# pierluigiferrari/ssd_keras

Measured on NVIDIA H100. Metric: SSD300 images/sec (fwd+decode), higher is better.
Workload: dtype bf16x3 (bf16 hi+lo operands, 3 wgmma MMAs per product, fp32 accumulate)

## Files before the change

include/ssdk.h:

```cpp
#ifndef SSDK_H_
#define SSDK_H_

#include <stddef.h>
#include <stdint.h>

#ifdef __cplusplus
extern "C" {
#endif

#define SSDK_VERSION 100

typedef enum {
  SSDK_OK = 0,
  SSDK_ERR_INVALID = -1,
  SSDK_ERR_CUDA = -2,
  SSDK_ERR_UNSUPPORTED = -3,
  SSDK_ERR_NOMEM = -4,
  SSDK_ERR_DEGENERATE = -5
} ssdk_status;

typedef enum { SSDK_COORDS_CENTROIDS = 0, SSDK_COORDS_CORNERS = 1, SSDK_COORDS_MINMAX = 2 } ssdk_coords;

typedef struct ssdk_ctx ssdk_ctx;
typedef struct ssdk_encoder ssdk_encoder;
// ... 150 lines not shown

typedef struct {
  int batch;
  int img_height, img_width, img_channels;
  int n_classes_total;
  int n_layers;
  const ssdk_layer_desc* layers;
  int precision;
  const float* anchors_f32;
  float variances[4];
  int training;
} ssdk_model_desc;

int ssdk_l2_normalize(ssdk_ctx* ctx, const float* x_dev, long long rows, int C, const float* gamma_dev, float* out_dev, void* stream);

int ssdk_conv2d_fwd(ssdk_ctx* ctx, const float* x_dev, int B, int H, int W, int Cin, const float* kernel_hwio_host,
                    const float* bias_host , int Cout, int kh, int kw, int stride, int dilation,
                    int pad_t, int pad_l, int pad_b, int pad_r, int act , int precision, float* y_dev, void* stream);
int ssdk_maxpool(ssdk_ctx* ctx, const float* x_dev, int B, int H, int W, int C, int kh, int kw, int stride,
                 int pad_t, int pad_l, int pad_b, int pad_r, float* y_dev, void* stream);

int ssdk_schedule_preview(int n_layers, const int* kind, const int* grid, const int* input, int R, int sm_count,
                          unsigned char* out_on_side, int* out_from, int* out_grid_cap);

int ssdk_model_create(ssdk_ctx* ctx, const ssdk_model_desc* desc, ssdk_model** out);
int ssdk_model_destroy(ssdk_model* m);
int ssdk_model_num_priors(const ssdk_model* m, int* out_P);
int ssdk_model_layer_shape(const ssdk_model* m, int layer, int* out_h, int* out_w, int* out_c);
int ssdk_model_forward(ssdk_model* m, const float* images_dev, float* y_pred_dev, void* stream);
int ssdk_model_read_layer(ssdk_model* m, int layer, float* out_dev, void* stream);
int ssdk_model_flops(const ssdk_model* m, double* out_algorithmic, double* out_issued);
int ssdk_model_set_timing(ssdk_model* m, int enable);
int ssdk_model_last_conv_ms(ssdk_model* m, float* out_ms);

enum ssdk_plan_kernel {
  SSDK_PLAN_NONE = 0,
  SSDK_PLAN_GEMM = 1,
  SSDK_PLAN_IM2COL_GEMM = 2,
  SSDK_PLAN_FIRST_TC = 3,
  SSDK_PLAN_DIRECT = 4
};
enum ssdk_plan_epilogue { SSDK_PLAN_EPI_SPLIT = 0, SSDK_PLAN_EPI_F32 = 1, SSDK_PLAN_EPI_ATOMIC = 2, SSDK_PLAN_EPI_HEAD = 3 };
typedef struct ssdk_layer_plan {
  int kernel;
  int bn;
  int split;
  int stages;
  int kblocks;
  int n_tiles_m, n_tiles_n;
  int grid;
  int k_split;
  int epilogue;
  int head_fused;
  int im2col_vec8;
} ssdk_layer_plan;
int ssdk_model_layer_plan(const ssdk_model* m, int layer, ssdk_layer_plan* out);

typedef struct ssdk_trainer ssdk_trainer;
int ssdk_trainer_create(ssdk_model* m, float* flat_grad_dev , ssdk_trainer** out);
int ssdk_trainer_destroy(ssdk_trainer* t);
int ssdk_trainer_num_params(const ssdk_trainer* t, long long* out_n);
int ssdk_trainer_param_span(const ssdk_trainer* t, int layer, int which, long long* out_offset, long long* out_count);
float* ssdk_trainer_grad_buffer(ssdk_trainer* t);
int ssdk_train_backward(ssdk_trainer* t, const float* y_true_dev, const float* y_pred_dev, int neg_pos_ratio, int n_neg_min,
                        float alpha, float* out_loss_dev , void* stream);
int ssdk_train_backward_begin(ssdk_trainer* t, const float* y_true_dev, const float* y_pred_dev, int neg_pos_ratio, int n_neg_min,
// ... 37 lines not shown
```

ssd_keras_b200/_ffi.py:

```python
import ctypes as C
import os
import threading

import numpy as np

_HERE = os.path.dirname(os.path.abspath(__file__))
_LIB_PATH = os.path.join(_HERE, '_lib', 'libssdk.so')

SSDK_OK = 0
SSDK_ERR_INVALID = -1
SSDK_ERR_CUDA = -2
SSDK_ERR_UNSUPPORTED = -3
SSDK_ERR_NOMEM = -4
SSDK_ERR_DEGENERATE = -5

COORDS = {'centroids': 0, 'corners': 1, 'minmax': 2}
BORDER_D = {'half': 0, 'include': 1, 'exclude': -1}

c_int_p = C.POINTER(C.c_int)
c_float_p = C.POINTER(C.c_float)
c_double_p = C.POINTER(C.c_double)


class AnchorCfg(C.Structure):
# ... 122 lines not shown
        L.ssdk_iou.argtypes = [vp, vp, C.c_int, vp, C.c_int, C.c_int, C.c_int, C.c_int, vp, vp]
        L.ssdk_decode.argtypes = [vp, C.POINTER(DecodeCfg), vp, C.c_int, vp, vp, vp, vp]
        L.ssdk_nms.argtypes = [vp, vp, vp, C.c_int, C.c_int, C.c_double, C.c_double, C.c_int, C.c_int, vp, vp, vp, vp]
        L.ssdk_ssd_loss_fwd.argtypes = [vp, vp, vp, C.c_int, C.c_int, C.c_int, C.c_int, C.c_int, C.c_float, vp, vp, vp]
        L.ssdk_ssd_loss_bwd.argtypes = [vp, vp, vp, C.c_int, C.c_int, C.c_int, C.c_int, C.c_int, C.c_float, vp, vp, vp]
        L.ssdk_ssd_loss_fwd_bwd.argtypes = [vp, vp, vp, C.c_int, C.c_int, C.c_int, C.c_int, C.c_int, C.c_float, vp, vp, vp, vp, vp]
        L.ssdk_ssd_loss_ws_layout.argtypes = [C.c_int, C.c_int, C.POINTER(LossWsLayout)]
        L.ssdk_ssd_loss_phase.argtypes = [vp, C.c_int, vp, vp, C.c_int, C.c_int, C.c_int, C.c_int, C.c_int, C.c_float, vp, C.c_int, vp,
                                          C.c_int, vp, vp, vp, vp, vp]
        for name in ('ssdk_ssd_loss_fwd_bwd', 'ssdk_ssd_loss_ws_layout', 'ssdk_ssd_loss_phase'):
            getattr(L, name).restype = C.c_int
        L.ssdk_eval_match.argtypes = [vp, C.c_int, vp, C.c_int, vp, vp, vp, vp, vp, vp, vp, vp, C.c_double, C.c_int, vp, vp, vp]
        L.ssdk_eval_cumsum.argtypes = [vp, vp, vp, vp, C.c_int, vp, vp, vp]
        L.ssdk_eval_match.restype = C.c_int
        L.ssdk_eval_cumsum.restype = C.c_int
        L.ssdk_assemble_batch.argtypes = [vp, vp, C.c_int, vp, C.c_int, C.c_int, vp, C.c_int, vp, vp, vp, vp]
        L.ssdk_assemble_batch.restype = C.c_int
        L.ssdk_l2_normalize.argtypes = [vp, vp, C.c_longlong, C.c_int, vp, vp, vp]
        L.ssdk_l2_normalize.restype = C.c_int
        L.ssdk_conv2d_fwd.argtypes = [vp, vp] + [C.c_int] * 4 + [vp, vp] + [C.c_int] * 11 + [vp, vp]
        L.ssdk_conv2d_fwd.restype = C.c_int
        L.ssdk_maxpool.argtypes = [vp, vp] + [C.c_int] * 11 + [vp, vp]
        L.ssdk_maxpool.restype = C.c_int
        if hasattr(L, 'ssdk_model_create'):
            L.ssdk_model_create.argtypes = [vp, C.POINTER(ModelDesc), C.POINTER(vp)]
            L.ssdk_model_destroy.argtypes = [vp]
            L.ssdk_model_num_priors.argtypes = [vp, c_int_p]
            L.ssdk_model_layer_shape.argtypes = [vp, C.c_int, c_int_p, c_int_p, c_int_p]
            L.ssdk_model_forward.argtypes = [vp, vp, vp, vp]
            L.ssdk_model_read_layer.argtypes = [vp, C.c_int, vp, vp]
            L.ssdk_model_flops.argtypes = [vp, c_double_p, c_double_p]
            L.ssdk_model_set_timing.argtypes = [vp, C.c_int]
            L.ssdk_model_last_conv_ms.argtypes = [vp, c_float_p]
            L.ssdk_model_layer_plan.argtypes = [vp, C.c_int, C.POINTER(LayerPlan)]
            L.ssdk_model_layer_plan.restype = C.c_int
        if hasattr(L, 'ssdk_trainer_create'):
            L.ssdk_trainer_create.argtypes = [vp, vp, C.POINTER(vp)]
            L.ssdk_trainer_destroy.argtypes = [vp]
            L.ssdk_trainer_num_params.argtypes = [vp, C.POINTER(C.c_longlong)]
            L.ssdk_trainer_param_span.argtypes = [vp, C.c_int, C.c_int, C.POINTER(C.c_longlong), C.POINTER(C.c_longlong)]
            L.ssdk_trainer_grad_buffer.argtypes = [vp]
            L.ssdk_trainer_grad_buffer.restype = vp
            L.ssdk_train_backward.argtypes = [vp, vp, vp, C.c_int, C.c_int, C.c_float, vp, vp]
            L.ssdk_train_apply_adam.argtypes = [vp, C.c_float, C.c_float, C.c_float, C.c_float, C.c_float, C.c_float, C.c_int, vp]
            L.ssdk_train_apply_adam.restype = C.c_int
            L.ssdk_trainer_read_bn_stats.argtypes = [vp, C.c_int, vp, vp, vp]
            L.ssdk_trainer_read_bn_stats.restype = C.c_int
            L.ssdk_train_backward_dy.argtypes = [vp, vp, vp]
            L.ssdk_train_backward_dy.restype = C.c_int
            L.ssdk_train_backward_begin.argtypes = [vp, vp, vp, C.c_int, C.c_int, C.c_float, vp, vp]
            L.ssdk_train_backward_begin.restype = C.c_int
            L.ssdk_train_backward_layers.argtypes = [vp, vp, C.c_int, C.c_int, vp]
            L.ssdk_train_backward_layers.restype = C.c_int
            L.ssdk_train_apply.argtypes = [vp, C.c_float, C.c_float, C.c_float, C.c_float, vp]
            L.ssdk_trainer_read_params.argtypes = [vp, vp, vp]
            L.ssdk_trainer_layer_plan.argtypes = [vp, C.c_int, C.POINTER(TrainerLayerPlan)]
            L.ssdk_trainer_layer_plan.restype = C.c_int
            for name in ('ssdk_trainer_create', 'ssdk_trainer_destroy', 'ssdk_trainer_num_params', 'ssdk_trainer_param_span',
                         'ssdk_train_backward', 'ssdk_train_apply', 'ssdk_trainer_read_params'):
                getattr(L, name).restype = C.c_int
        for name in ('ssdk_ctx_create', 'ssdk_ctx_destroy', 'ssdk_anchors_count', 'ssdk_anchors_generate',
                     'ssdk_encoder_create', 'ssdk_encoder_destroy', 'ssdk_encode', 'ssdk_encode_f64', 'ssdk_encode_dev', 'ssdk_iou_matrix', 'ssdk_iou', 'ssdk_decode',
                     'ssdk_nms', 'ssdk_ssd_loss_fwd', 'ssdk_ssd_loss_bwd'):
            getattr(L, name).restype = C.c_int
        _lib = L
    return _lib
# ... 87 lines not shown
```

ssd_keras_b200/csrc/conv.cu:

```cuda
#include "conv.cuh"
#include "tc.cuh"
#include <cudaTypedefs.h>
#include <cmath>
#include <cstdlib>
#include <cstring>
#include <algorithm>
#include <vector>

namespace ssdk {

static PFN_cuTensorMapEncodeTiled_v12000 g_encode = nullptr;

int tma_init() {
  if (g_encode) return SSDK_OK;
  void* fn = nullptr;
  cudaDriverEntryPointQueryResult qres;
  SSDK_CHECK_CUDA(cudaGetDriverEntryPoint("cuTensorMapEncodeTiled", &fn, cudaEnableDefault, &qres));
  if (qres != cudaDriverEntryPointSuccess || !fn) { set_error("cuTensorMapEncodeTiled is not available in this driver"); return SSDK_ERR_CUDA; }
  g_encode = reinterpret_cast<PFN_cuTensorMapEncodeTiled_v12000>(fn);
  return SSDK_OK;
}

int make_tmap_2d(CUtensorMap* out, const void* base, uint64_t inner, uint64_t rows, uint64_t row_stride_bytes,
                 uint32_t box_inner, uint32_t box_rows) {
// ... 84 lines not shown
    constexpr int kMaxCol = 256;
    const int c_lo = bx * CP4;
    const int k_lo = c_lo >> 5, k_hi = (c_lo + CP4 - 1) >> 5;
    if (c_lo + CP4 > kMaxCol) break;
    float v0[32], v1[32];
    ld_acc32(arow + k_lo * 32, v0);
    if (k_hi != k_lo) ld_acc32(arow + k_hi * 32, v1);
    float e[CP4];
#pragma unroll
    for (int r = 0; r < CP4; ++r) {
      const int col = c_lo + r;
      e[r] = (((col >> 5) == k_lo) ? v0[col & 31] : v1[col & 31]) + s_bias[col];
    }
    float mx = e[0];
#pragma unroll
    for (int r = 1; r < C; ++r) mx = fmaxf(mx, e[r]);
    float sum = 0.f;
#pragma unroll
    for (int r = 0; r < C; ++r) { e[r] = expf(e[r] - mx); sum += e[r]; }
    const float inv = 1.0f / sum;
    const int prior = args.head_prior_off + pix * args.head_nb + bx;
    float* dst = args.out_f32 + ((size_t)n * args.head_P + prior) * RW;
    const float4 an = __ldg(reinterpret_cast<const float4*>(args.head_anchors) + prior);
#pragma unroll
    for (int r = 0; r < C; ++r) dst[r] = e[r] * inv;
#pragma unroll
    for (int r = C; r < CP4; ++r) dst[r] = e[r];
    dst[C + 4] = an.x; dst[C + 5] = an.y; dst[C + 6] = an.z; dst[C + 7] = an.w;
    dst[C + 8] = args.head_var[0]; dst[C + 9] = args.head_var[1]; dst[C + 10] = args.head_var[2]; dst[C + 11] = args.head_var[3];
  }
}

template <bool BWD>
__device__ __forceinline__ void epi_split(const ConvArgs& args, const float* acc, int ncols, size_t o, const float* sb,
                                          const float* ss, const float* sh) {
  if (!BWD && !args.bn_scale && args.act == SSDK_ACT_RELU && args.out_lo) {
    for (int c0 = 0; c0 < ncols; c0 += 32) {
      float vr[32];
      ld_acc32(acc + c0, vr);
#pragma unroll
      for (int g2 = 0; g2 < 2; ++g2) {
        uint32_t ph[8], pl[8];
#pragma unroll
        for (int h = 0; h < 2; ++h) {
          const int g = g2 * 2 + h;
          if (c0 + g * 8 < ncols) {
            const float4 b0 = *reinterpret_cast<const float4*>(sb + c0 + g * 8);
            const float4 b1 = *reinterpret_cast<const float4*>(sb + c0 + g * 8 + 4);
            const float bb[8] = {b0.x, b0.y, b0.z, b0.w, b1.x, b1.y, b1.z, b1.w};
#pragma unroll
            for (int j = 0; j < 4; ++j) {
              const float f0 = fmaxf(vr[g * 8 + j * 2] + bb[j * 2], 0.f);
              const float f1 = fmaxf(vr[g * 8 + j * 2 + 1] + bb[j * 2 + 1], 0.f);
              const __nv_bfloat162 hh = __floats2bfloat162_rn(f0, f1);
              const uint32_t hp = *reinterpret_cast<const uint32_t*>(&hh);
              const __nv_bfloat162 ll = __floats2bfloat162_rn(f0 - __uint_as_float(hp << 16), f1 - __uint_as_float(hp & 0xffff0000u));
              ph[h * 4 + j] = hp; pl[h * 4 + j] = *reinterpret_cast<const uint32_t*>(&ll);
            }
          }
        }
        const int cA = c0 + g2 * 16;
        {
          if (cA < ncols) {
            *reinterpret_cast<uint4*>(args.out_hi + o + cA) = make_uint4(ph[0], ph[1], ph[2], ph[3]);
            *reinterpret_cast<uint4*>(args.out_lo + o + cA) = make_uint4(pl[0], pl[1], pl[2], pl[3]);
          }
          if (cA + 8 < ncols) {
            *reinterpret_cast<uint4*>(args.out_hi + o + cA + 8) = make_uint4(ph[4], ph[5], ph[6], ph[7]);
            *reinterpret_cast<uint4*>(args.out_lo + o + cA + 8) = make_uint4(pl[4], pl[5], pl[6], pl[7]);
          }
        }
      }
    }
    return;
  }
  for (int c0 = 0; c0 < ncols; c0 += 32) {
    float vr[32];
    ld_acc32(acc + c0, vr);
#pragma unroll
    for (int g = 0; g < 4; ++g) {
      if (c0 + g * 8 < ncols) {
        uint32_t ph[4], pl[4];
        uint4 mk = make_uint4(0x3f803f80u, 0x3f803f80u, 0x3f803f80u, 0x3f803f80u), oh = make_uint4(0, 0, 0, 0), ol = oh;
        if (BWD) {
          if (args.mask_hi) mk = *reinterpret_cast<const uint4*>(args.mask_hi + o + c0 + g * 8);
          if (args.accumulate) {
            oh = *reinterpret_cast<const uint4*>(args.out_hi + o + c0 + g * 8);
            if (args.out_lo) ol = *reinterpret_cast<const uint4*>(args.out_lo + o + c0 + g * 8);
          }
        }
        const uint32_t mkw[4] = {mk.x, mk.y, mk.z, mk.w}, ohw[4] = {oh.x, oh.y, oh.z, oh.w}, olw[4] = {ol.x, ol.y, ol.z, ol.w};
#pragma unroll
        for (int j = 0; j < 4; ++j) {
          float f[2];
#pragma unroll
          for (int e = 0; e < 2; ++e) {
            const int col = c0 + g * 8 + j * 2 + e;
            float xv = vr[g * 8 + j * 2 + e] + sb[col];
            if (args.bn_scale) xv = xv * ss[col] + sh[col];
            xv = apply_act(xv, args.act);
            if (BWD) {
              if (!(__uint_as_float(((mkw[j] >> (e * 16)) & 0xffffu) << 16) > 0.f)) xv = 0.f;
              xv += __uint_as_float(((ohw[j] >> (e * 16)) & 0xffffu) << 16) + __uint_as_float(((olw[j] >> (e * 16)) & 0xffffu) << 16);
            }
            f[e] = xv;
          }
          __nv_bfloat16 h0 = __float2bfloat16_rn(f[0]), h1 = __float2bfloat16_rn(f[1]);
          __nv_bfloat16 l0 = __float2bfloat16_rn(f[0] - __bfloat162float(h0));
          __nv_bfloat16 l1 = __float2bfloat16_rn(f[1] - __bfloat162float(h1));
          ph[j] = (uint32_t)__bfloat16_as_ushort(h0) | ((uint32_t)__bfloat16_as_ushort(h1) << 16);
          pl[j] = (uint32_t)__bfloat16_as_ushort(l0) | ((uint32_t)__bfloat16_as_ushort(l1) << 16);
        }
        *reinterpret_cast<uint4*>(args.out_hi + o + c0 + g * 8) = make_uint4(ph[0], ph[1], ph[2], ph[3]);
        if (args.out_lo) *reinterpret_cast<uint4*>(args.out_lo + o + c0 + g * 8) = make_uint4(pl[0], pl[1], pl[2], pl[3]);
      }
    }
  }
}

enum { kSingle = 0, kSplitXS = 2 };
template <int BN, int MODE>
__global__ void __launch_bounds__(256, 1)
conv_wgmma_kernel(const __grid_constant__ CUtensorMap tm_a_hi, const __grid_constant__ CUtensorMap tm_a_lo,
                  const __grid_constant__ CUtensorMap tm_b_hi, const __grid_constant__ CUtensorMap tm_b_lo,
                  const __grid_constant__ ConvArgs args) {
  extern __shared__ unsigned char smem_dyn[];
  const uint32_t smem_base = (smem_u32(smem_dyn) + 1023u) & ~1023u;
  unsigned char* smem_al = smem_dyn + (smem_base - smem_u32(smem_dyn));
  const int tid = threadIdx.x, wg = tid >> 7, warp = tid >> 5, lane = tid & 31;
  constexpr bool split = MODE == kSplitXS;
  const int S = args.stages;
  constexpr uint32_t kBTile = (uint32_t)BN * kBK * 2;
  const uint32_t b_off = (uint32_t)kATile * (split ? 2u : 1u);
  const uint32_t stage = b_off + kBTile * (split ? 2u : 1u);
  const uint32_t ring = max(stage * (uint32_t)S, ((uint32_t)kBM * (BN + kAccPad) + 32u) * 4u);
  const uint32_t bar_base = smem_base + ring;
  auto full = [&](uint32_t s) { return bar_base + 8u * s; };
  auto empty = [&](uint32_t s) { return bar_base + 8u * ((uint32_t)S + s); };
  float* s_acc = reinterpret_cast<float*>(smem_al);
  float* s_bias = reinterpret_cast<float*>(smem_al + ring + 256);
  float* s_scale = s_bias + BN;
  float* s_shift = s_scale + BN;

  if (tid == 0) {
    prefetch_tmap(&tm_a_hi); prefetch_tmap(&tm_b_hi);
    if (split) { prefetch_tmap(&tm_a_lo); prefetch_tmap(&tm_b_lo); }
    for (int s = 0; s < S; ++s) { mbar_init(full(s), 1); mbar_init(empty(s), 8); }
    asm volatile("fence.mbarrier_init.release.cluster;" ::: "memory");
  }
  __syncthreads();

  const int KS = args.k_split > 1 ? args.k_split : 1;
  const int total_tiles = args.n_tiles_m * args.n_tiles_n * KS;
  uint32_t g = 0;
  float acc[BN / 2], accx[split ? BN / 2 : 1];
  for (int t = blockIdx.x; t < total_tiles; t += gridDim.x) {
    const int tt = t / KS, ks = t - tt * KS;
    const int m0 = args.tile_list[tt / args.n_tiles_n] * kBM;
    const int n0 = (tt % args.n_tiles_n) * BN;
    const int kb0 = KS > 1 ? ks * args.kb_per : 0;
    const int kb1 = KS > 1 ? min(args.kblocks, kb0 + args.kb_per) : args.kblocks;
    const int nkb = kb1 - kb0, nk = args.KH * args.KW * nkb;
    for (int i = tid; i < BN; i += blockDim.x) {
      const int col = n0 + i;
      s_bias[i] = (args.bias && col < args.cout) ? args.bias[col] : 0.f;
      if (args.bn_scale) { s_scale[i] = col < args.cout ? args.bn_scale[col] : 0.f; s_shift[i] = col < args.cout ? args.bn_shift[col] : 0.f; }
    }
    auto issue = [&](int i) {
      const uint32_t gi = g + (uint32_t)i, s = gi % (uint32_t)S;
      mbar_wait(empty(s), ((gi / (uint32_t)S) & 1u) ^ 1u);
      const int tap = i / nkb, kb = kb0 + (i - tap * nkb), kh = tap / args.KW, kw = tap - kh * args.KW;
      const int row = m0 + args.row_shift[kh] + kw * args.kw_rows;
      const int kcol = (tap * args.kblocks + kb) * kBK + args.b_k_offset;
      const uint32_t dst = smem_base + stage * s;
      mbar_expect_tx(full(s), stage);
      tma_load_2d(dst, &tm_a_hi, kb * kBK, row, full(s));
      tma_load_2d(dst + b_off, &tm_b_hi, kcol, n0, full(s));
      if (split) {
        tma_load_2d(dst + kATile, &tm_a_lo, kb * kBK, row, full(s));
        tma_load_2d(dst + b_off + kBTile, &tm_b_lo, kcol, n0, full(s));
      }
    };
    auto release = [&](int j) {
      __syncwarp();
      if (lane == 0) mbar_arrive(empty((g + (uint32_t)j) % (uint32_t)S));
      if (tid == 0 && j + S < nk) issue(j + S);
    };
    if (tid == 0)
      for (int i = 0; i < min(S, nk); ++i) issue(i);
    wgmma_fence_acc(acc);
    wgmma_fence_acc(accx);
    for (int i = 0; i < nk; ++i) {
      const uint32_t gi = g + (uint32_t)i, s = gi % (uint32_t)S;
      mbar_wait(full(s), (gi / (uint32_t)S) & 1u);
      const uint32_t a_hi = smem_base + stage * s + (uint32_t)wg * (kATile / 2), b_hi = smem_base + stage * s + b_off;
      constexpr uint64_t kDesc = wgmma_desc_hi(16);
      wgmma_fence();
#pragma unroll
      for (int k = 0; k < 4; ++k) {
        const uint32_t sc = (i | k) ? 1u : 0u;
        const uint64_t da = wgmma_desc(kDesc, a_hi + 32u * k), db = wgmma_desc(kDesc, b_hi + 32u * k);
        Wgmma<BN, 0, 0>::mma(acc, da, db, sc);
        if constexpr (split) {
          Wgmma<BN, 0, 0>::mma(accx, da, wgmma_desc(kDesc, b_hi + kBTile + 32u * k), sc);
          Wgmma<BN, 0, 0>::mma(accx, wgmma_desc(kDesc, a_hi + kATile + 32u * k), db, 1u);
        }
      }
      wgmma_commit();
      wgmma_wait<1>();
      if (i > 0) release(i - 1);
    }
    wgmma_wait<0>();
    wgmma_fence_acc(acc);
    wgmma_fence_acc(accx);
    if (nk > 0) release(nk - 1);
    g += (uint32_t)nk;
    if constexpr (split) {
#pragma unroll
      for (int j = 0; j < BN / 2; ++j) acc[j] += accx[j];
    }

    __syncthreads();
    store_acc_tile<BN>(acc, s_acc, wg, warp, lane);
    __syncthreads();
    const int r = tid & (kBM - 1), half = tid >> 7;
    const int v = m0 + r;
    bool valid = v < args.M_total;
    int n = 0, y = 0, x = 0;
    if (valid) {
      n = v / args.rows_per_img;
      const int rr = v - n * args.rows_per_img;
      y = rr / args.in_Wp;
      x = rr - y * args.in_Wp;
      valid = (y < args.Ho) && (x < args.Wo);
    }
    const float* arow = s_acc + (size_t)r * (BN + kAccPad);
    const int ncols = min(BN, args.cout - n0);
    const int h0 = half * (BN / 2), nh = min(BN / 2, ncols - h0);
    if (valid && args.epi == EPI_HEAD) {
      if (half == 0) {
        const int C = args.head_C, CP4 = C + 4, RW = C + 12;
        const int pix = y * args.Wo + x;
        if (CP4 == 25 && args.head_nb <= 8) {
          epi_head_fixed<25>(args, arow, n, pix, s_bias);
        } else {
          for (int bx = 0; bx < args.head_nb; ++bx) {
            const int c_lo = bx * CP4;
            float mx = -INFINITY;
            for (int c = c_lo; c < c_lo + C; ++c) mx = fmaxf(mx, arow[c] + s_bias[c]);
            float sum = 0.f;
            for (int c = c_lo; c < c_lo + C; ++c) sum += expf(arow[c] + s_bias[c] - mx);
            const int prior = args.head_prior_off + pix * args.head_nb + bx;
            float* dst = args.out_f32 + ((size_t)n * args.head_P + prior) * RW;
            for (int rc = 0; rc < CP4; ++rc) {
              const float val = arow[c_lo + rc] + s_bias[c_lo + rc];
              dst[rc] = rc < C ? expf(val - mx) / sum : val;
            }
            const float4 an = __ldg(reinterpret_cast<const float4*>(args.head_anchors) + prior);
            dst[C + 4] = an.x; dst[C + 5] = an.y; dst[C + 6] = an.z; dst[C + 7] = an.w;
            dst[C + 8] = args.head_var[0]; dst[C + 9] = args.head_var[1]; dst[C + 10] = args.head_var[2]; dst[C + 11] = args.head_var[3];
          }
        }
      }
    } else if (valid && nh > 0) {
      if (args.epi == EPI_SPLIT) {
        const size_t o = (((size_t)n * args.out_Hp + (y + args.out_pad)) * args.out_Wp + (x + args.out_pad)) * args.out_Cs + n0 + h0;
        if (args.mask_hi || args.accumulate) epi_split<true>(args, arow + h0, nh, o, s_bias + h0, s_scale + h0, s_shift + h0);
        else epi_split<false>(args, arow + h0, nh, o, s_bias + h0, s_scale + h0, s_shift + h0);
      } else if (args.epi == EPI_ATOMIC) {
        float* dstp = args.out_f32 + (size_t)v * args.out_ld + args.out_col_off + n0 + h0;
        for (int j = 0; j < nh; ++j) atomicAdd(dstp + j, arow[h0 + j]);
      } else {
        const size_t o = (((size_t)n * args.Ho + y) * args.Wo + x) * (size_t)args.cout + n0 + h0;
        for (int j = 0; j < nh; ++j) args.out_f32[o + j] = apply_act(arow[h0 + j] + s_bias[h0 + j], args.act);
      }
    }
    fence_proxy_async();
    __syncthreads();
  }
}

template <int BN, int MODE>
static int launch_conv_bn(const ConvLaunch& L, int grid, cudaStream_t stream) {
  static bool attr_set = false;
  if (!attr_set) {
    SSDK_CHECK_CUDA(cudaFuncSetAttribute(conv_wgmma_kernel<BN, MODE>, cudaFuncAttributeMaxDynamicSharedMemorySize, 227 * 1024));
    attr_set = true;
  }
  conv_wgmma_kernel<BN, MODE><<<grid, 256, L.smem, stream>>>(L.a_hi, L.a_lo, L.b_hi, L.b_lo, L.args);
  return SSDK_OK;
}

int launch_conv(ssdk_ctx* ctx, const ConvLaunch& L, cudaStream_t stream, int grid_cap) {
  const int grid = grid_cap > 0 ? std::max(1, std::min(L.grid, grid_cap)) : L.grid;
  const bool split = L.args.split != 0;
  SSDK_REQUIRE(!split || L.args.acc_split, "internal: bf16x3 conv plans carry the cross-term accumulator");
  SSDK_REQUIRE(split || L.args.BN != 160, "internal: 160-wide conv tiles are for bf16x3 predictor heads");
  int rc;
  switch (L.args.BN) {
    case 64: rc = split ? launch_conv_bn<64, kSplitXS>(L, grid, stream) : launch_conv_bn<64, kSingle>(L, grid, stream); break;
    case 128: rc = split ? launch_conv_bn<128, kSplitXS>(L, grid, stream) : launch_conv_bn<128, kSingle>(L, grid, stream); break;
    case 160: rc = launch_conv_bn<160, kSplitXS>(L, grid, stream); break;
    case 256:
      SSDK_REQUIRE(!split, "internal: 256-wide conv tiles have no cross-term accumulator");
      rc = launch_conv_bn<256, kSingle>(L, grid, stream);
      break;
    default: set_error("internal: conv tile width %d", L.args.BN); return SSDK_ERR_INVALID;
  }
  if (rc) return rc;
  SSDK_COUNT_LAUNCH(ctx);
  SSDK_CHECK_CUDA(cudaGetLastError());
  return SSDK_OK;
}

__device__ __forceinline__ void split_store(const ActBuf& o, size_t idx, float v) {
  __nv_bfloat16 h = __float2bfloat16_rn(v);
  o.hi[idx] = h;
  if (o.lo) o.lo[idx] = __float2bfloat16_rn(v - __bfloat162float(h));
}
__device__ __forceinline__ float split_load(const ActBuf& a, size_t idx) {
  float v = __bfloat162float(a.hi[idx]);
  if (a.lo) v += __bfloat162float(a.lo[idx]);
// ... 304 lines not shown
            const uint32_t off = (uint32_t)(tap >> 4) * kATile + (uint32_t)r * 128u + ((uint32_t)(((tap >> 1) & 7) ^ (r & 7)) << 4) + (uint32_t)(tap & 1) * 8u;
            *reinterpret_cast<uint2*>(a_dst + off) = w[j];
          }
        }
      }
    }
    fence_proxy_async();
    __syncthreads();
    {
      constexpr uint64_t kDesc = wgmma_desc_hi(16);
      wgmma_fence_acc(acc);
      wgmma_fence();
#pragma unroll
      for (int ks = 0; ks < KB * 4; ++ks) {
        const int kb = ks >> 2, k = ks & 3;
        const uint32_t ah = a_base + (uint32_t)kb * kATile + (uint32_t)wg * (kATile / 2) + 32u * k;
        const uint32_t bh = b_base + (uint32_t)kb * b_block + 32u * k;
        const uint64_t da = wgmma_desc(kDesc, ah), db = wgmma_desc(kDesc, bh);
        Wgmma<BN, 0, 0>::mma(acc, da, db, ks ? 1u : 0u);
        if constexpr (split) {
          Wgmma<BN, 0, 0>::mma(acc, da, wgmma_desc(kDesc, bh + b_plane), 1u);
          Wgmma<BN, 0, 0>::mma(acc, wgmma_desc(kDesc, ah + a_plane), db, 1u);
        }
      }
      wgmma_commit();
      wgmma_wait<0>();
      wgmma_fence_acc(acc);
    }
    store_acc_tile<BN>(acc, s_acc, wg, warp, lane);
    __syncthreads();
    const int h0 = plane * (BN / 2), nh = min(BN / 2, fa.epi.cout - h0);
    if (valid && nh > 0) {
      const size_t o = (((size_t)n * fa.epi.out_Hp + (y + fa.epi.out_pad)) * fa.epi.out_Wp + (x + fa.epi.out_pad)) * fa.epi.out_Cs + h0;
      epi_split<false>(fa.epi, s_acc + (size_t)r * (BN + kAccPad) + h0, nh, o, s_bias + h0, s_scale + h0, s_shift + h0);
    }
    __syncthreads();
  }
}

void first_weight_image(const float* hwio, int taps, int cin, int cout, int BN, int kblocks, std::vector<uint16_t>& hi, std::vector<uint16_t>& lo) {
  hi.assign((size_t)kblocks * BN * 64, 0); lo.assign((size_t)kblocks * BN * 64, 0);
  auto f2bf = [](float f) { uint32_t u; memcpy(&u, &f, 4); if ((u & 0x7f800000u) == 0x7f800000u) return (uint16_t)(u >> 16);
                            u += 0x7fffu + ((u >> 16) & 1u); return (uint16_t)(u >> 16); };
  auto bf2f = [](uint16_t h) { uint32_t u = (uint32_t)h << 16; float f; memcpy(&f, &u, 4); return f; };
  for (int o = 0; o < cout; ++o)
    for (int t = 0; t < taps; ++t)
      for (int c = 0; c < cin; ++c) {
        const int k = t * 4 + c, kb = k >> 6, kk = k & 63;
        const size_t byte = (size_t)kb * BN * 128 + (size_t)o * 128 + ((size_t)((kk >> 3) ^ (o & 7)) << 4) + (size_t)(kk & 7) * 2;
        const float w = hwio[((size_t)t * cin + c) * cout + o];
        const uint16_t h = f2bf(w);
        hi[byte / 2] = h; lo[byte / 2] = f2bf(w - bf2f(h));
      }
}

bool first_border_ok(const ActBuf& in, int kh, int kw, int dil, int pad_t, int pad_l) {
  return in.pad >= pad_t && in.pad >= pad_l && in.pad >= (kh - 1) * dil - pad_t && in.pad >= (kw - 1) * dil - pad_l;
}
int first_tc_supported(int taps, int cin, int cout) { return cin <= 4 && taps * 4 <= 128 && cout % 8 == 0 && cout <= 128; }

template <int BN, int KB, bool SPLIT>
static int launch_first_bn(const FirstArgs& fa, int grid, size_t smem, cudaStream_t stream) {
  static bool attr_set = false;
  if (!attr_set) {
    SSDK_CHECK_CUDA(cudaFuncSetAttribute(conv_first_kernel<BN, KB, SPLIT>, cudaFuncAttributeMaxDynamicSharedMemorySize, 227 * 1024));
    attr_set = true;
  }
// ... 307 lines not shown
```

ssd_keras_b200/csrc/model.cu:

```cuda
#include "model.cuh"

using namespace ssdk;

namespace {

void pack_weights(const LayerPlan& L, int cin, int cout, int taps, int kblocks, bool im2col, int Ctot,
                  std::vector<uint16_t>& hi, std::vector<uint16_t>& lo, std::vector<float>& bias) {
  const ssdk_layer_desc& d = L.d;
  const size_t Krow = im2col ? (size_t)kblocks * 64 : (size_t)taps * kblocks * 64;
  hi.assign((size_t)cout * Krow, 0); lo.assign((size_t)cout * Krow, 0);
  bias.assign(cout, 0.f);
  const bool head = d.op == SSDK_OP_HEAD;
  const int nb = d.n_boxes;
  const int c_conf = head ? nb * Ctot : cout;
  const int c_loc = head ? nb * 4 : 0;
  for (int o = 0; o < cout; ++o) {
    const float* ker; int oc, ocn;
    if (!head) { ker = d.kernel; oc = o; ocn = c_conf; bias[o] = d.bias ? d.bias[o] : 0.f; }
    else {
      const int b = o / (Ctot + 4), r = o % (Ctot + 4);
      if (r < Ctot) { ker = d.kernel; oc = b * Ctot + r; ocn = c_conf; bias[o] = d.bias ? d.bias[oc] : 0.f; }
      else { ker = d.kernel2; oc = b * 4 + (r - Ctot); ocn = c_loc; bias[o] = d.bias2 ? d.bias2[oc] : 0.f; }
    }
    for (int t = 0; t < taps; ++t)
// ... 424 lines not shown
  const ConvArgs& a = L.launch.args;
  out->kernel = L.im2col ? SSDK_PLAN_IM2COL_GEMM : SSDK_PLAN_GEMM;
  out->bn = a.BN; out->split = a.split; out->stages = a.stages; out->kblocks = a.kblocks;
  out->n_tiles_m = a.n_tiles_m; out->n_tiles_n = a.n_tiles_n; out->grid = L.launch.grid; out->k_split = a.k_split > 1 ? a.k_split : 1;
  out->epilogue = a.epi; out->head_fused = L.head_fused ? 1 : 0;
  out->im2col_vec8 = L.im2col && L.im2col_vec8 ? 1 : 0;
  return SSDK_OK;
}

extern "C" int ssdk_model_flops(const ssdk_model* m, double* algo, double* issued) {
  SSDK_REQUIRE(m, "ssdk_model_flops: NULL model");
  if (algo) *algo = m->flops_algo;
  if (issued) *issued = m->flops_issued;
  return SSDK_OK;
}

extern "C" int ssdk_model_set_timing(ssdk_model* m, int enable) {
  SSDK_REQUIRE(m, "ssdk_model_set_timing: NULL model");
  m->timing = enable ? 1 : 0;
  return SSDK_OK;
}

extern "C" int ssdk_model_last_conv_ms(ssdk_model* m, float* out_ms) {
  SSDK_REQUIRE(m && out_ms, "ssdk_model_last_conv_ms: NULL argument");
  float total = 0.f;
  for (auto& L : m->layers) {
    if (!L.ev0 || L.direct) continue;
    SSDK_CHECK_CUDA(cudaEventSynchronize(L.ev1));
    float ms = 0.f;
    SSDK_CHECK_CUDA(cudaEventElapsedTime(&ms, L.ev0, L.ev1));
    total += ms;
  }
  *out_ms = total;
  return SSDK_OK;
}

extern "C" int ssdk_model_forward(ssdk_model* m, const float* images_dev, float* y_pred_dev, void* stream_) {
  SSDK_REQUIRE(m && images_dev, "ssdk_model_forward: NULL argument");
  SSDK_REQUIRE(m->P == 0 || y_pred_dev, "ssdk_model_forward: y_pred_dev is NULL");
  cudaStream_t main_stream = (cudaStream_t)stream_;
  ssdk_ctx* ctx = m->ctx;
  int rc;
  const bool overlap = m->overlap_from >= 0 && !m->timing;
  int issued[2] = {0, 0}, seen[2] = {0, 0}, side_used = 0;
  std::vector<int>& pos = m->issue_pos;
  pos.assign(m->layers.size(), 0);
  for (size_t i = 0; i < m->layers.size(); ++i) {
    LayerPlan& L = m->layers[i];
    const ssdk_layer_desc& d = L.d;
    const int sx = overlap && m->on_side[i] ? 1 : 0;
    cudaStream_t stream = sx ? m->side : main_stream;
    int cap = 0;
    if (overlap) {
      if (d.op != SSDK_OP_INPUT && d.input >= 0) {
        const int sy = m->on_side[d.input] ? 1 : 0;
        const bool first_side = sx == 1 && !side_used;
        if ((sy != sx && pos[d.input] > seen[sx]) || first_side) {
          cudaStream_t other = sx ? main_stream : m->side;
          SSDK_CHECK_CUDA(cudaEventRecord(m->dep_ev[i], other));
          SSDK_CHECK_CUDA(cudaStreamWaitEvent(stream, m->dep_ev[i], 0));
          seen[sx] = issued[sx ^ 1];
        }
      }
      if (sx) side_used = 1;
      pos[i] = ++issued[sx];
      if (!sx && side_used) cap = m->grid_cap;
// ... 135 lines not shown
```

ssd_keras_b200/models/_graph.py:

```python
import ctypes as C

import numpy as np

from .. import _ffi
from ..keras_layers.keras_layer_DecodeDetections import DecodeDetections
from ..keras_layers.keras_layer_DecodeDetectionsFast import DecodeDetectionsFast
from ._keras_api import KerasTrainingMixin


class _LayerInfo:
    def __init__(self, name, output_shape):
        self.name = name
        self.output_shape = output_shape


class Spec:

    def __init__(self, name, op, inp=None, cout=0, k=(1, 1), stride=1, dilation=1, pad=(0, 0, 0, 0), act=_ffi.ACT_NONE,
                 n_boxes=0, bn=None, params=None):
        self.name, self.op, self.inp, self.cout = name, op, inp, cout
        self.kh, self.kw = k
        self.stride, self.dilation, self.pad, self.act, self.n_boxes = stride, dilation, pad, act, n_boxes
        self.bn = bn
        self.params = params or {}
# ... 390 lines not shown
                yield item[0] if isinstance(item, (tuple, list)) else item
        outs = [r.numpy().copy() for r in self.predict_stream(images())]
        if not outs:
            raise ValueError('predict_generator: the generator yielded no batch')
        return np.concatenate(outs, axis=0)

    def predict(self, x, batch_size=None):
        x = np.asarray(x, dtype=np.float32)
        bs = batch_size or x.shape[0]
        outs = [r.numpy().copy() for r in self.predict_stream(x[i:i + bs] for i in range(0, x.shape[0], bs))]
        return np.concatenate(outs, axis=0)

    def read_layer(self, name, batch):
        import torch
        i = self.index[name]
        h, w, c = self._shapes[i]
        out = torch.empty((batch, h, w, c), dtype=torch.float32, device='cuda')
        _ffi.check(_ffi.lib().ssdk_model_read_layer(self._plan(batch)['handle'], i, _ffi.dptr(out), _ffi.stream_ptr()))
        return out.cpu().numpy()

    def flops(self, batch):
        a, b = C.c_double(), C.c_double()
        _ffi.check(_ffi.lib().ssdk_model_flops(self._plan(batch)['handle'], C.byref(a), C.byref(b)))
        return a.value, b.value

    def set_timing(self, batch, enable=True):
        _ffi.check(_ffi.lib().ssdk_model_set_timing(self._plan(batch)['handle'], 1 if enable else 0))

    def last_conv_ms(self, batch):
        v = C.c_float()
        _ffi.check(_ffi.lib().ssdk_model_last_conv_ms(self._plan(batch)['handle'], C.byref(v)))
        return v.value


def resolve_box_args(n_predictor_layers, min_scale, max_scale, scales, aspect_ratios_global, aspect_ratios_per_layer,
                     two_boxes_for_ar1, steps, offsets, variances):
    if aspect_ratios_global is None and aspect_ratios_per_layer is None:
        raise ValueError("`aspect_ratios_global` and `aspect_ratios_per_layer` cannot both be None. At least one needs to be specified.")
    if aspect_ratios_per_layer:
        if len(aspect_ratios_per_layer) != n_predictor_layers:
            raise ValueError("It must be either aspect_ratios_per_layer is None or len(aspect_ratios_per_layer) == {}, but "
                             "len(aspect_ratios_per_layer) == {}.".format(n_predictor_layers, len(aspect_ratios_per_layer)))
    if (min_scale is None or max_scale is None) and scales is None:
        raise ValueError("Either `min_scale` and `max_scale` or `scales` need to be specified.")
    if scales:
        if len(scales) != n_predictor_layers + 1:
            raise ValueError("It must be either scales is None or len(scales) == {}, but len(scales) == {}."
                             .format(n_predictor_layers + 1, len(scales)))
    else:
        scales = np.linspace(min_scale, max_scale, n_predictor_layers + 1)
    if len(variances) != 4:
        raise ValueError("4 variance values must be pased, but {} values were received.".format(len(variances)))
    variances = np.array(variances)
    if np.any(variances <= 0):
        raise ValueError("All variances must be >0, but the variances given are {}".format(variances))
    if (steps is not None) and (len(steps) != n_predictor_layers):
        raise ValueError("You must provide at least one step value per predictor layer.")
    if (offsets is not None) and (len(offsets) != n_predictor_layers):
        raise ValueError("You must provide at least one offset value per predictor layer.")
    if aspect_ratios_per_layer:
        aspect_ratios = aspect_ratios_per_layer
    else:
        aspect_ratios = [aspect_ratios_global] * n_predictor_layers
    n_boxes = [len(ar) + (1 if (1 in ar) and two_boxes_for_ar1 else 0) for ar in aspect_ratios]
    return scales, aspect_ratios, n_boxes, variances
```

Before: 1622.

## Warp-specialize conv wgmma kernel with producer warpgroup and register-direct split epilogue

Adds a dedicated TMA producer warpgroup (384 threads, setmaxnreg rebalancing) so loads are issued independently of the two consumer warpgroups. For the split bf16 epilogue, consumers now write outputs straight from registers using quad shuffles instead of staging the accumulator through shared memory with block-wide barriers. Staged epilogues use a named consumer barrier plus an mbarrier to hold the producer back until the shared accumulator is free. A per-layer timing query API is also added. The risks are higher register pressure in the consumers, extra shuffle and load work in the epilogue, and less overlap for the staged path.

```diff
diff --git a/include/ssdk.h b/include/ssdk.h
--- a/include/ssdk.h
+++ b/include/ssdk.h
@@ -206,6 +206,7 @@
 int ssdk_model_flops(const ssdk_model* m, double* out_algorithmic, double* out_issued);
 int ssdk_model_set_timing(ssdk_model* m, int enable);
 int ssdk_model_last_conv_ms(ssdk_model* m, float* out_ms);
+int ssdk_model_layer_ms(const ssdk_model* m, int layer, float* out_ms);
 
 enum ssdk_plan_kernel {
   SSDK_PLAN_NONE = 0,
diff --git a/ssd_keras_b200/_ffi.py b/ssd_keras_b200/_ffi.py
--- a/ssd_keras_b200/_ffi.py
+++ b/ssd_keras_b200/_ffi.py
@@ -178,6 +178,7 @@
             L.ssdk_model_flops.argtypes = [vp, c_double_p, c_double_p]
             L.ssdk_model_set_timing.argtypes = [vp, C.c_int]
             L.ssdk_model_last_conv_ms.argtypes = [vp, c_float_p]
+            L.ssdk_model_layer_ms.argtypes = [vp, C.c_int, c_float_p]
             L.ssdk_model_layer_plan.argtypes = [vp, C.c_int, C.POINTER(LayerPlan)]
             L.ssdk_model_layer_plan.restype = C.c_int
         if hasattr(L, 'ssdk_trainer_create'):
diff --git a/ssd_keras_b200/csrc/conv.cu b/ssd_keras_b200/csrc/conv.cu
--- a/ssd_keras_b200/csrc/conv.cu
+++ b/ssd_keras_b200/csrc/conv.cu
@@ -140,9 +140,46 @@
 }
 
 template <bool BWD>
+__device__ __forceinline__ void epi_split8(const ConvArgs& args, const float* v, size_t o, const float* sb, const float* ss,
+                                           const float* sh) {
+  uint32_t ph[4], pl[4];
+  uint4 mk = make_uint4(0x3f803f80u, 0x3f803f80u, 0x3f803f80u, 0x3f803f80u), oh = make_uint4(0, 0, 0, 0), ol = oh;
+  if (BWD) {
+    if (args.mask_hi) mk = *reinterpret_cast<const uint4*>(args.mask_hi + o);
+    if (args.accumulate) {
+      oh = *reinterpret_cast<const uint4*>(args.out_hi + o);
+      if (args.out_lo) ol = *reinterpret_cast<const uint4*>(args.out_lo + o);
+    }
+  }
+  const uint32_t mkw[4] = {mk.x, mk.y, mk.z, mk.w}, ohw[4] = {oh.x, oh.y, oh.z, oh.w}, olw[4] = {ol.x, ol.y, ol.z, ol.w};
+#pragma unroll
+  for (int j = 0; j < 4; ++j) {
+    float f[2];
+#pragma unroll
+    for (int e = 0; e < 2; ++e) {
+      const int col = j * 2 + e;
+      float xv = v[col] + sb[col];
+      if (args.bn_scale) xv = xv * ss[col] + sh[col];
+      xv = apply_act(xv, args.act);
+      if (BWD) {
+        if (!(__uint_as_float(((mkw[j] >> (e * 16)) & 0xffffu) << 16) > 0.f)) xv = 0.f;
+        xv += __uint_as_float(((ohw[j] >> (e * 16)) & 0xffffu) << 16) + __uint_as_float(((olw[j] >> (e * 16)) & 0xffffu) << 16);
+      }
+      f[e] = xv;
+    }
+    __nv_bfloat16 h0 = __float2bfloat16_rn(f[0]), h1 = __float2bfloat16_rn(f[1]);
+    __nv_bfloat16 l0 = __float2bfloat16_rn(f[0] - __bfloat162float(h0));
+    __nv_bfloat16 l1 = __float2bfloat16_rn(f[1] - __bfloat162float(h1));
+    ph[j] = (uint32_t)__bfloat16_as_ushort(h0) | ((uint32_t)__bfloat16_as_ushort(h1) << 16);
+    pl[j] = (uint32_t)__bfloat16_as_ushort(l0) | ((uint32_t)__bfloat16_as_ushort(l1) << 16);
+  }
+  *reinterpret_cast<uint4*>(args.out_hi + o) = make_uint4(ph[0], ph[1], ph[2], ph[3]);
+  if (args.out_lo) *reinterpret_cast<uint4*>(args.out_lo + o) = make_uint4(pl[0], pl[1], pl[2], pl[3]);
+}
+
 __device__ __forceinline__ void epi_split(const ConvArgs& args, const float* acc, int ncols, size_t o, const float* sb,
                                           const float* ss, const float* sh) {
-  if (!BWD && !args.bn_scale && args.act == SSDK_ACT_RELU && args.out_lo) {
+  if (!args.bn_scale && args.act == SSDK_ACT_RELU && args.out_lo) {
     for (int c0 = 0; c0 < ncols; c0 += 32) {
       float vr[32];
       ld_acc32(acc + c0, vr);
@@ -186,56 +223,45 @@
     float vr[32];
     ld_acc32(acc + c0, vr);
 #pragma unroll
-    for (int g = 0; g < 4; ++g) {
-      if (c0 + g * 8 < ncols) {
-        uint32_t ph[4], pl[4];
-        uint4 mk = make_uint4(0x3f803f80u, 0x3f803f80u, 0x3f803f80u, 0x3f803f80u), oh = make_uint4(0, 0, 0, 0), ol = oh;
-        if (BWD) {
-          if (args.mask_hi) mk = *reinterpret_cast<const uint4*>(args.mask_hi + o + c0 + g * 8);
-          if (args.accumulate) {
-            oh = *reinterpret_cast<const uint4*>(args.out_hi + o + c0 + g * 8);
-            if (args.out_lo) ol = *reinterpret_cast<const uint4*>(args.out_lo + o + c0 + g * 8);
-          }
-        }
-        const uint32_t mkw[4] = {mk.x, mk.y, mk.z, mk.w}, ohw[4] = {oh.x, oh.y, oh.z, oh.w}, olw[4] = {ol.x, ol.y, ol.z, ol.w};
-#pragma unroll
-        for (int j = 0; j < 4; ++j) {
-          float f[2];
-#pragma unroll
-          for (int e = 0; e < 2; ++e) {
-            const int col = c0 + g * 8 + j * 2 + e;
-            float xv = vr[g * 8 + j * 2 + e] + sb[col];
-            if (args.bn_scale) xv = xv * ss[col] + sh[col];
-            xv = apply_act(xv, args.act);
-            if (BWD) {
-              if (!(__uint_as_float(((mkw[j] >> (e * 16)) & 0xffffu) << 16) > 0.f)) xv = 0.f;
-              xv += __uint_as_float(((ohw[j] >> (e * 16)) & 0xffffu) << 16) + __uint_as_float(((olw[j] >> (e * 16)) & 0xffffu) << 16);
-            }
-            f[e] = xv;
-          }
-          __nv_bfloat16 h0 = __float2bfloat16_rn(f[0]), h1 = __float2bfloat16_rn(f[1]);
-          __nv_bfloat16 l0 = __float2bfloat16_rn(f[0] - __bfloat162float(h0));
-          __nv_bfloat16 l1 = __float2bfloat16_rn(f[1] - __bfloat162float(h1));
-          ph[j] = (uint32_t)__bfloat16_as_ushort(h0) | ((uint32_t)__bfloat16_as_ushort(h1) << 16);
-          pl[j] = (uint32_t)__bfloat16_as_ushort(l0) | ((uint32_t)__bfloat16_as_ushort(l1) << 16);
-        }
-        *reinterpret_cast<uint4*>(args.out_hi + o + c0 + g * 8) = make_uint4(ph[0], ph[1], ph[2], ph[3]);
-        if (args.out_lo) *reinterpret_cast<uint4*>(args.out_lo + o + c0 + g * 8) = make_uint4(pl[0], pl[1], pl[2], pl[3]);
-      }
-    }
+    for (int g = 0; g < 4; ++g)
+      if (c0 + g * 8 < ncols) epi_split8<false>(args, vr + g * 8, o + c0 + g * 8, sb + c0 + g * 8, ss + c0 + g * 8, sh + c0 + g * 8);
   }
 }
 
 enum { kSingle = 0, kSplitXS = 2 };
+static constexpr int kConvThreads = 384;
+
+__device__ __forceinline__ void consumer_sync() { asm volatile("bar.sync 1, 256;" ::: "memory"); }
+
+template <int N>
+__device__ __forceinline__ void quad_gather8(const float (&acc)[N], int jp, int q, float (&v)[8]) {
+  const float2 c00 = make_float2(acc[4 * jp], acc[4 * jp + 1]), c01 = make_float2(acc[4 * jp + 2], acc[4 * jp + 3]);
+  const float2 c10 = make_float2(acc[4 * jp + 4], acc[4 * jp + 5]), c11 = make_float2(acc[4 * jp + 6], acc[4 * jp + 7]);
+  float2 rcv[4];
+#pragma unroll
+  for (int r = 0; r < 4; ++r) {
+    const int u = q ^ r;
+    const float2 s = (u & 1) ? ((u & 2) ? c11 : c10) : ((u & 2) ? c01 : c00);
+    rcv[r].x = __shfl_xor_sync(0xffffffffu, s.x, r);
+    rcv[r].y = __shfl_xor_sync(0xffffffffu, s.y, r);
+  }
+#pragma unroll
+  for (int p = 0; p < 4; ++p) {
+    const int r = q ^ p;
+    const float2 t = r == 0 ? rcv[0] : (r == 1 ? rcv[1] : (r == 2 ? rcv[2] : rcv[3]));
+    v[2 * p] = t.x; v[2 * p + 1] = t.y;
+  }
+}
+
 template <int BN, int MODE>
-__global__ void __launch_bounds__(256, 1)
+__global__ void __launch_bounds__(kConvThreads, 1)
 conv_wgmma_kernel(const __grid_constant__ CUtensorMap tm_a_hi, const __grid_constant__ CUtensorMap tm_a_lo,
                   const __grid_constant__ CUtensorMap tm_b_hi, const __grid_constant__ CUtensorMap tm_b_lo,
                   const __grid_constant__ ConvArgs args) {
   extern __shared__ unsigned char smem_dyn[];
   const uint32_t smem_base = (smem_u32(smem_dyn) + 1023u) & ~1023u;
   unsigned char* smem_al = smem_dyn + (smem_base - smem_u32(smem_dyn));
-  const int tid = threadIdx.x, wg = tid >> 7, warp = tid >> 5, lane = tid & 31;
+  const int tid = threadIdx.x, wg = tid >> 7, lane = tid & 31;
   constexpr bool split = MODE == kSplitXS;
   const int S = args.stages;
   constexpr uint32_t kBTile = (uint32_t)BN * kBK * 2;
@@ -245,63 +271,91 @@
   const uint32_t bar_base = smem_base + ring;
   auto full = [&](uint32_t s) { return bar_base + 8u * s; };
   auto empty = [&](uint32_t s) { return bar_base + 8u * ((uint32_t)S + s); };
+  const uint32_t staged_free = bar_base + 16u * (uint32_t)S;
   float* s_acc = reinterpret_cast<float*>(smem_al);
   float* s_bias = reinterpret_cast<float*>(smem_al + ring + 256);
   float* s_scale = s_bias + BN;
   float* s_shift = s_scale + BN;
+  const bool staged = args.epi != EPI_SPLIT;
 
   if (tid == 0) {
     prefetch_tmap(&tm_a_hi); prefetch_tmap(&tm_b_hi);
     if (split) { prefetch_tmap(&tm_a_lo); prefetch_tmap(&tm_b_lo); }
     for (int s = 0; s < S; ++s) { mbar_init(full(s), 1); mbar_init(empty(s), 8); }
+    mbar_init(staged_free, 1);
     asm volatile("fence.mbarrier_init.release.cluster;" ::: "memory");
   }
   __syncthreads();
 
   const int KS = args.k_split > 1 ? args.k_split : 1;
   const int total_tiles = args.n_tiles_m * args.n_tiles_n * KS;
+  auto unit = [&](int t, int& m0, int& n0, int& kb0, int& nkb) {
+    const int tt = t / KS, ks = t - tt * KS;
+    m0 = args.tile_list[tt / args.n_tiles_n] * kBM;
+    n0 = (tt % args.n_tiles_n) * BN;
+    kb0 = KS > 1 ? ks * args.kb_per : 0;
+    const int kb1 = KS > 1 ? min(args.kblocks, kb0 + args.kb_per) : args.kblocks;
+    nkb = kb1 - kb0;
+  };
+
+  if (wg == 0) {
+    asm volatile("setmaxnreg.dec.sync.aligned.u32 40;");
+    if (tid != 0) return;
+    uint32_t g = 0;
+    uint32_t lt = 0;
+    for (int t = blockIdx.x; t < total_tiles; t += gridDim.x, ++lt) {
+      int m0, n0, kb0, nkb;
+      unit(t, m0, n0, kb0, nkb);
+      const int nk = args.KH * args.KW * nkb;
+      if (staged && lt > 0) mbar_wait(staged_free, (lt - 1) & 1u);
+      for (int i = 0; i < nk; ++i) {
+        const uint32_t gi = g + (uint32_t)i, s = gi % (uint32_t)S;
+        mbar_wait(empty(s), ((gi / (uint32_t)S) & 1u) ^ 1u);
+        const int tap = i / nkb, kb = kb0 + (i - tap * nkb), kh = tap / args.KW, kw = tap - kh * args.KW;
+        const int row = m0 + args.row_shift[kh] + kw * args.kw_rows;
+        const int kcol = (tap * args.kblocks + kb) * kBK + args.b_k_offset;
+        const uint32_t dst = smem_base + stage * s;
+        mbar_expect_tx(full(s), stage);
+        tma_load_2d(dst, &tm_a_hi, kb * kBK, row, full(s));
+        tma_load_2d(dst + b_off, &tm_b_hi, kcol, n0, full(s));
+        if (split) {
+          tma_load_2d(dst + kATile, &tm_a_lo, kb * kBK, row, full(s));
+          tma_load_2d(dst + b_off + kBTile, &tm_b_lo, kcol, n0, full(s));
+        }
+      }
+      g += (uint32_t)nk;
+    }
+    return;
+  }
+
+  asm volatile("setmaxnreg.inc.sync.aligned.u32 232;");
+  const int cw = wg - 1, ctid = tid - 128, cwarp = (tid >> 5) & 3;
   uint32_t g = 0;
   float acc[BN / 2], accx[split ? BN / 2 : 1];
   for (int t = blockIdx.x; t < total_tiles; t += gridDim.x) {
-    const int tt = t / KS, ks = t - tt * KS;
-    const int m0 = args.tile_list[tt / args.n_tiles_n] * kBM;
-    const int n0 = (tt % args.n_tiles_n) * BN;
-    const int kb0 = KS > 1 ? ks * args.kb_per : 0;
-    const int kb1 = KS > 1 ? min(args.kblocks, kb0 + args.kb_per) : args.kblocks;
-    const int nkb = kb1 - kb0, nk = args.KH * args.KW * nkb;
-    for (int i = tid; i < BN; i += blockDim.x) {
-      const int col = n0 + i;
-      s_bias[i] = (args.bias && col < args.cout) ? args.bias[col] : 0.f;
-      if (args.bn_scale) { s_scale[i] = col < args.cout ? args.bn_scale[col] : 0.f; s_shift[i] = col < args.cout ? args.bn_shift[col] : 0.f; }
-    }
-    auto issue = [&](int i) {
-      const uint32_t gi = g + (uint32_t)i, s = gi % (uint32_t)S;
-      mbar_wait(empty(s), ((gi / (uint32_t)S) & 1u) ^ 1u);
-      const int tap = i / nkb, kb = kb0 + (i - tap * nkb), kh = tap / args.KW, kw = tap - kh * args.KW;
-      const int row = m0 + args.row_shift[kh] + kw * args.kw_rows;
-      const int kcol = (tap * args.kblocks + kb) * kBK + args.b_k_offset;
-      const uint32_t dst = smem_base + stage * s;
-      mbar_expect_tx(full(s), stage);
-      tma_load_2d(dst, &tm_a_hi, kb * kBK, row, full(s));
-      tma_load_2d(dst + b_off, &tm_b_hi, kcol, n0, full(s));
-      if (split) {
-        tma_load_2d(dst + kATile, &tm_a_lo, kb * kBK, row, full(s));
-        tma_load_2d(dst + b_off + kBTile, &tm_b_lo, kcol, n0, full(s));
-      }
-    };
+    int m0, n0, kb0, nkb;
+    unit(t, m0, n0, kb0, nkb);
+    const int nk = args.KH * args.KW * nkb;
+    if (staged)
+      for (int i = ctid; i < BN; i += 256) {
+        const int col = n0 + i;
+        s_bias[i] = (args.bias && col < args.cout) ? args.bias[col] : 0.f;
+        if (args.bn_scale) { s_scale[i] = col < args.cout ? args.bn_scale[col] : 0.f; s_shift[i] = col < args.cout ? args.bn_shift[col] : 0.f; }
+      }
     auto release = [&](int j) {
       __syncwarp();
       if (lane == 0) mbar_arrive(empty((g + (uint32_t)j) % (uint32_t)S));
-      if (tid == 0 && j + S < nk) issue(j + S);
     };
-    if (tid == 0)
-      for (int i = 0; i < min(S, nk); ++i) issue(i);
+#pragma unroll
+    for (int j = 0; j < BN / 2; ++j) acc[j] = 0.f;
+#pragma unroll
+    for (int j = 0; j < (split ? BN / 2 : 1); ++j) accx[j] = 0.f;
     wgmma_fence_acc(acc);
     wgmma_fence_acc(accx);
     for (int i = 0; i < nk; ++i) {
       const uint32_t gi = g + (uint32_t)i, s = gi % (uint32_t)S;
       mbar_wait(full(s), (gi / (uint32_t)S) & 1u);
-      const uint32_t a_hi = smem_base + stage * s + (uint32_t)wg * (kATile / 2), b_hi = smem_base + stage * s + b_off;
+      const uint32_t a_hi = smem_base + stage * s + (uint32_t)cw * (kATile / 2), b_hi = smem_base + stage * s + b_off;
       constexpr uint64_t kDesc = wgmma_desc_hi(16);
       wgmma_fence();
 #pragma unroll
@@ -327,11 +381,48 @@
 #pragma unroll
       for (int j = 0; j < BN / 2; ++j) acc[j] += accx[j];
     }
-
-    __syncthreads();
-    store_acc_tile<BN>(acc, s_acc, wg, warp, lane);
-    __syncthreads();
-    const int r = tid & (kBM - 1), half = tid >> 7;
+    const int ncols = min(BN, args.cout - n0);
+
+    if (!staged) {
+      const int q = lane & 3;
+      const int v = m0 + cw * 64 + cwarp * 16 + (lane >> 2) + 8 * (q >> 1);
+      bool valid = v < args.M_total;
+      int n = 0, y = 0, x = 0;
+      if (valid) {
+        n = v / args.rows_per_img;
+        const int rr = v - n * args.rows_per_img;
+        y = rr / args.in_Wp;
+        x = rr - y * args.in_Wp;
+        valid = (y < args.Ho) && (x < args.Wo);
+      }
+      const size_t o_row = (((size_t)n * args.out_Hp + (y + args.out_pad)) * args.out_Wp + (x + args.out_pad)) * args.out_Cs + n0;
+      const bool bwd = args.mask_hi || args.accumulate;
+#pragma unroll
+      for (int jp = 0; jp < BN / 8; jp += 2) {
+        float vr[8];
+        quad_gather8(acc, jp, q, vr);
+        const int c0 = 8 * (jp + (q & 1));
+        if (valid && c0 < ncols) {
+          float sb[8], ss[8], sh[8];
+#pragma unroll
+          for (int e = 0; e < 8; ++e) {
+            const int col = n0 + c0 + e;
+            const bool in = col < args.cout;
+            sb[e] = (args.bias && in) ? __ldg(args.bias + col) : 0.f;
+            ss[e] = (args.bn_scale && in) ? __ldg(args.bn_scale + col) : 0.f;
+            sh[e] = (args.bn_scale && in) ? __ldg(args.bn_shift + col) : 0.f;
+          }
+          if (bwd) epi_split8<true>(args, vr, o_row + c0, sb, ss, sh);
+          else epi_split8<false>(args, vr, o_row + c0, sb, ss, sh);
+        }
+      }
+      continue;
+    }
+
+    consumer_sync();
+    store_acc_tile<BN>(acc, s_acc, cw, cwarp, lane);
+    consumer_sync();
+    const int r = ctid & (kBM - 1), half = ctid >> 7;
     const int v = m0 + r;
     bool valid = v < args.M_total;
     int n = 0, y = 0, x = 0;
@@ -343,7 +434,6 @@
       valid = (y < args.Ho) && (x < args.Wo);
     }
     const float* arow = s_acc + (size_t)r * (BN + kAccPad);
-    const int ncols = min(BN, args.cout - n0);
     const int h0 = half * (BN / 2), nh = min(BN / 2, ncols - h0);
     if (valid && args.epi == EPI_HEAD) {
       if (half == 0) {
@@ -371,11 +461,7 @@
         }
       }
     } else if (valid && nh > 0) {
-      if (args.epi == EPI_SPLIT) {
-        const size_t o = (((size_t)n * args.out_Hp + (y + args.out_pad)) * args.out_Wp + (x + args.out_pad)) * args.out_Cs + n0 + h0;
-        if (args.mask_hi || args.accumulate) epi_split<true>(args, arow + h0, nh, o, s_bias + h0, s_scale + h0, s_shift + h0);
-        else epi_split<false>(args, arow + h0, nh, o, s_bias + h0, s_scale + h0, s_shift + h0);
-      } else if (args.epi == EPI_ATOMIC) {
+      if (args.epi == EPI_ATOMIC) {
         float* dstp = args.out_f32 + (size_t)v * args.out_ld + args.out_col_off + n0 + h0;
         for (int j = 0; j < nh; ++j) atomicAdd(dstp + j, arow[h0 + j]);
       } else {
@@ -384,7 +470,8 @@
       }
     }
     fence_proxy_async();
-    __syncthreads();
+    consumer_sync();
+    if (ctid == 0) mbar_arrive(staged_free);
   }
 }
 
@@ -395,7 +482,7 @@
     SSDK_CHECK_CUDA(cudaFuncSetAttribute(conv_wgmma_kernel<BN, MODE>, cudaFuncAttributeMaxDynamicSharedMemorySize, 227 * 1024));
     attr_set = true;
   }
-  conv_wgmma_kernel<BN, MODE><<<grid, 256, L.smem, stream>>>(L.a_hi, L.a_lo, L.b_hi, L.b_lo, L.args);
+  conv_wgmma_kernel<BN, MODE><<<grid, kConvThreads, L.smem, stream>>>(L.a_hi, L.a_lo, L.b_hi, L.b_lo, L.args);
   return SSDK_OK;
 }
 
@@ -766,7 +853,7 @@
     const int h0 = plane * (BN / 2), nh = min(BN / 2, fa.epi.cout - h0);
     if (valid && nh > 0) {
       const size_t o = (((size_t)n * fa.epi.out_Hp + (y + fa.epi.out_pad)) * fa.epi.out_Wp + (x + fa.epi.out_pad)) * fa.epi.out_Cs + h0;
-      epi_split<false>(fa.epi, s_acc + (size_t)r * (BN + kAccPad) + h0, nh, o, s_bias + h0, s_scale + h0, s_shift + h0);
+      epi_split(fa.epi, s_acc + (size_t)r * (BN + kAccPad) + h0, nh, o, s_bias + h0, s_scale + h0, s_shift + h0);
     }
     __syncthreads();
   }
diff --git a/ssd_keras_b200/csrc/model.cu b/ssd_keras_b200/csrc/model.cu
--- a/ssd_keras_b200/csrc/model.cu
+++ b/ssd_keras_b200/csrc/model.cu
@@ -480,6 +480,16 @@
     total += ms;
   }
   *out_ms = total;
+  return SSDK_OK;
+}
+
+extern "C" int ssdk_model_layer_ms(const ssdk_model* m, int layer, float* out_ms) {
+  SSDK_REQUIRE(m && out_ms && layer >= 0 && layer < (int)m->layers.size(), "ssdk_model_layer_ms: bad argument");
+  const LayerPlan& L = m->layers[layer];
+  *out_ms = 0.f;
+  if (!L.ev0 || L.direct) return SSDK_OK;
+  SSDK_CHECK_CUDA(cudaEventSynchronize(L.ev1));
+  SSDK_CHECK_CUDA(cudaEventElapsedTime(out_ms, L.ev0, L.ev1));
   return SSDK_OK;
 }
 
diff --git a/ssd_keras_b200/models/_graph.py b/ssd_keras_b200/models/_graph.py
--- a/ssd_keras_b200/models/_graph.py
+++ b/ssd_keras_b200/models/_graph.py
@@ -446,6 +446,14 @@
         _ffi.check(_ffi.lib().ssdk_model_last_conv_ms(self._plan(batch)['handle'], C.byref(v)))
         return v.value
 
+    def layer_ms(self, batch, name):
+        v = C.c_float()
+        _ffi.check(_ffi.lib().ssdk_model_layer_ms(self._plan(batch)['handle'], self.index[name], C.byref(v)))
+        return v.value
+
+    def layer_plan(self, batch, name):
+        return _ffi.model_layer_plan(self._plan(batch)['handle'], self.index[name])
+
 
 def resolve_box_args(n_predictor_layers, min_scale, max_scale, scales, aspect_ratios_global, aspect_ratios_per_layer,
                      two_boxes_for_ar1, steps, offsets, variances):
```

Result: faster. 1838 (median of 6 runs) (+13.3%).
